# markokr/libacm

Measured on AMD Instinct MI355X. Metric: decoded PCM Msamples/sec over a batch of ACM streams (hot path on HBM-resident staged input), higher is better.
Workload: dtype int32

## Files before the change

libacm_amd/csrc/acm_kernels.hip:

```cpp
#include <hip/hip_runtime.h>

#include <utility>

#include "acm_device.h"
#include "acm_late_scale.h"
#include "acm_kernel_geo.h"

#ifndef ACM_L14_GROUPS
#define ACM_L14_GROUPS 3, 3, 3, 3, 2
#endif
#ifndef ACM_L13_GROUPS
#define ACM_L13_GROUPS 2, 3, 3, 3, 2
#endif

#ifndef ACM_OUT_F32
#define ACM_OUT_F32 0
#endif
#if ACM_OUT_F32
#define ACM_K_EMIT acm_sw_emit_f32
#define ACM_K_SMALL acm_small_level_f32
#define ACM_K_FUSED acm_fused_tile_f32
#define ACM_K_TILE2 acm_f32_tile2
#define ACM_K_CHUNK acm_f32_chunk
#define ACMK_OUT(name) name##_f32
// ... 1950 lines not shown
	struct Desc { uint32_t e[NE]; };
	struct Tables {
		v4i_t coef[3][NM][64];
		int32_t bias[3][2][QN];
		int32_t rsum[3][QN];
	};

	static __device__ __forceinline__ void fill_tables(Tables &t, const int tid, const int nthreads)
	{
		constexpr int32_t ONE = 1 << OutScale<L>::SHIFT;
		for (int k = tid; k < 3 * NM * 64; k += nthreads) {
			const int j = k / (NM * 64), mt = (k / 64) % NM, lane = k % 64;
			t.coef[j][mt][lane] = *reinterpret_cast<const v4i_t *>(&ACM_TZ6[VARIANT][j][16 * mt + (lane & 15)][16 * (lane >> 4)]);
		}
		for (int k = tid; k < 3 * 2 * QN; k += nthreads) {
			const int var = k / (2 * QN), par = (k / QN) & 1, q = k % QN;
			t.bias[var][par][q] = par ? 0 : ACM_TZ6_BIAS[VARIANT][var][q] * ONE;
		}
		for (int k = tid; k < 3 * QN; k += nthreads) {
			int32_t sum = 0;
			for (int c = 0; c < 64; c++)
				sum += ACM_TZ6[VARIANT][k / QN][k % QN][c];
			t.rsum[k / QN][k % QN] = 128 * sum;
		}
	}

	static __device__ __forceinline__ Desc fetch_desc(const uint32_t *__restrict__ pairs, const AcmTile2 &r)
	{
		Desc d;
		const uint32_t at = __builtin_amdgcn_readfirstlane((uint32_t)r.idx_off);
#pragma unroll
		for (int j = 0; j < NE; j++)
			d.e[j] = pairs[at + j];
		return d;
	}

	static __device__ __forceinline__ uint32_t entry_of(const Desc &d, const uint32_t u)
	{
		uint32_t e = (uint32_t)opaque_s((int32_t)d.e[0]);
#pragma unroll
		for (int j = 1; j < NE; j++)
			e = (u >> 1) >= (uint32_t)j ? (uint32_t)opaque_s((int32_t)d.e[j]) : e;
		return e;
	}

	template <int CTRL, int BANKS>
	static __device__ __forceinline__ v4u_t dpp4(const v4u_t old, const v4u_t src)
	{
		v4u_t r;
#pragma unroll
		for (int v = 0; v < 4; v++)
			r[v] = (uint32_t)__builtin_amdgcn_update_dpp((int)old[v], (int)src[v], CTRL, 0xF, BANKS, false);
		return r;
	}
	static constexpr int DPP_W0_BANKS = (1 << (SIGMA / 4)) - 1;
	static __device__ __forceinline__ void hand_history_on(Raw &raw)
	{
#pragma unroll
		for (int k = 0; k < 2; k++) {
			raw.lo[0][k] = dpp4<0x100 + (16 - SIGMA), DPP_W0_BANKS>(raw.lo[0][k], raw.lo[0][k + NSW]);
			raw.hi[0][k] = dpp4<0x100 + (16 - SIGMA), DPP_W0_BANKS>(raw.hi[0][k], raw.hi[0][k + NSW]);
		}
	}
	static __device__ __forceinline__ void take_history_from_partner(Raw &raw)
	{
#pragma unroll
		for (int k = 0; k < 2; k++) {
			raw.lo[0][k] = dpp4<0x110 + SIGMA, 0xF & ~DPP_W0_BANKS>(raw.lo[0][k], raw.lo[0][k + NSW]);
			raw.hi[0][k] = dpp4<0x110 + SIGMA, 0xF & ~DPP_W0_BANKS>(raw.hi[0][k], raw.hi[0][k + NSW]);
		}
	}
	static constexpr int JM = (TR & 1) ? 1 : TR / 2;
	static_assert(JM + 1 <= NE, "entries in reach are entries fetched");
	static __device__ __forceinline__ uint32_t half_bytes(const uint32_t cls) { return (0x4234u >> (4u * cls)) & 15u; }
	template <int J0>
	static __device__ __forceinline__ uint32_t mode_of(const uint32_t flags, const Desc &d, const uint32_t sval)
	{
		const uint32_t cls = d.e[0] & 3u;
		const uint32_t pair_units = (uint32_t)(COLS / 64) * half_bytes(cls);
		bool ok = (flags & ACM_TILE_ONEBLOCK) != 0 && cls != 0u;
		if constexpr (OutScale<L>::SHIFT != 0)
			ok = ok && sval < 65536u;
#pragma unroll
		for (int j = 1; j <= JM; j++)
			ok = ok && (d.e[j] & 3u) == cls;
#pragma unroll
		for (int j = J0; j < JM; j++)
			ok = ok && (d.e[j + 1] >> 2) - (d.e[j] >> 2) == pair_units;
		return ok ? (cls == ACMHIP_BP_NIB12 ? 3u : cls - (ACMHIP_BP_BYTE - 1u)) : 0u;
	}

#ifndef ACM_K3_LD_MOD
#define ACM_K3_LD_MOD " nt"
#endif
	template <bool KEEP>
	static __device__ __forceinline__ void issue(Raw &raw, const uint8_t *arena, const Desc &d, const int lane, const uint32_t odd, const uint32_t mode)
	{
		static_assert(!KEEP || KEEPS_ROWS, "the rows in front belong to another lane");
		constexpr int K0 = KEEP ? 2 : 0, J0 = KEEP ? 1 : 0;
		const uint32_t i = (uint32_t)lane & 15u, ks = (uint32_t)lane >> 4;
		const uint32_t c = class_of(i), rr = RR == 1 ? 0u : i / SIGMA;
		const uint32_t smode = __builtin_amdgcn_readfirstlane(mode);
		uint32_t va[NX][NG], vh[NX][NG];
		const uint8_t *sb[NX][NG];
		if (mode) {
			const uint32_t hb = smode == 1u ? 2u : smode == 2u ? 4u : 3u;
			const uint64_t base = reinterpret_cast<uint64_t>(arena) + ((uint64_t)(d.e[J0] >> 2) << 6);
			const uint32_t vl = (rr * (uint32_t)(NSW * COLS / 2) + c * (uint32_t)(QN / 2)) * hb + 16u * ks;
			const uint32_t vlh = vl - (smode == 3u ? 8u * ks : 0u);
#pragma unroll
			for (int k = K0; k < NX; k++)
#pragma unroll
				for (int g = 0; g < NG; g++) {
					va[k][g] = vl;
					vh[k][g] = vlh;
					sb[k][g] = sgpr_u64(base + (uint64_t)((((TR & 1 ? odd : 0u) + (uint32_t)(k - K0)) * (uint32_t)(COLS / 2) + group_at(g) * (uint32_t)(QN / 2)) * hb));
				}
		} else {
			const uint32_t e0 = d.e[0];
			const uint8_t *base = sgpr_u64(reinterpret_cast<uint64_t>(arena) + ((uint64_t)(e0 >> 2) << 6));
#pragma unroll
			for (int k = K0; k < NX; k++) {
				const uint32_t u = (TR & 1 ? odd : 0u) + rr * NSW + k;
				const uint32_t e = entry_of(d, u);
				const uint32_t hb = half_bytes(e & 3u);
				const uint32_t row_at = (((e >> 2) - (e0 >> 2)) << 6) + ((u & 1u) ? (uint32_t)(COLS / 2) * hb : 0u) + 16u * ks;
#pragma unroll
				for (int g = 0; g < NG; g++) {
					va[k][g] = row_at + (group_at(g) + c) * (uint32_t)(QN / 2) * hb;
					vh[k][g] = va[k][g] - ((e & 3u) == ACMHIP_BP_NIB12 ? 8u * ks : 0u);
					sb[k][g] = base;
				}
			}
		}
#pragma unroll
		for (int k = K0; k < NX; k++)
#pragma unroll
			for (int g = 0; g < NG; g++) {
				if constexpr (KEEPS_ROWS) {
					asm volatile("global_load_dwordx4 %0, %1, %2" ACM_K3_LD_MOD : "=v"(raw.lo[g][k]) : "v"(va[k][g]), "s"(sb[k][g]) : "memory");
					asm volatile("s_cmp_eq_u32 %3, 1\n\ts_cbranch_scc1 .Lacm_z8_%=\n\t"
						     "global_load_dwordx4 %0, %1, %2 offset:64" ACM_K3_LD_MOD "\n"
						     ".Lacm_z8_%=:"
						     : "+v"(raw.hi[g][k]) : "v"(vh[k][g]), "s"(sb[k][g]), "s"(smode) : "memory", "scc");
				} else {
					asm volatile("global_load_dwordx4 %0, %1, %2" : "=v"(raw.lo[g][k]) : "v"(va[k][g]), "s"(sb[k][g]) : "memory");
					asm volatile("s_cmp_eq_u32 %3, 1\n\ts_cbranch_scc1 .Lacm_z8_%=\n\t"
						     "global_load_dwordx4 %0, %1, %2 offset:64\n"
						     ".Lacm_z8_%=:"
						     : "+v"(raw.hi[g][k]) : "v"(vh[k][g]), "s"(sb[k][g]), "s"(smode) : "memory", "scc");
				}
			}
	}
	static __device__ __forceinline__ v4u_t expand_nib(const v4u_t x)
	{
		const uint32_t M = 0xF0F0F0F0u;
		return v4u_t{ x[0] & M, (x[0] << 4) & M, x[1] & M, (x[1] << 4) & M };
	}
	static __device__ __forceinline__ v4u_t sra4(const v4u_t x)
	{
		v4u_t r;
#pragma unroll
		for (int v = 0; v < 4; v++) {
			const uint32_t m = x[v] & 0x80808080u;
			r[v] = ((x[v] >> 4) & 0x0F0F0F0Fu) | ((m << 1) - (m >> 3));
		}
		return r;
	}
	static __device__ __forceinline__ v4u_t shl4(const v4u_t x)
	{
		return v4u_t{ (x[0] << 4) & 0xF0F0F0F0u, (x[1] << 4) & 0xF0F0F0F0u, (x[2] << 4) & 0xF0F0F0F0u, (x[3] << 4) & 0xF0F0F0F0u };
	}
	static __device__ __forceinline__ void shift_history(Raw &raw)
	{
#pragma unroll
		for (int g = 0; g < NG; g++)
#pragma unroll
			for (int k = 0; k < 2; k++) {
				raw.lo[g][k] = raw.lo[g][k + NSW];
				raw.hi[g][k] = raw.hi[g][k + NSW];
			}
	}
	static __device__ __forceinline__ void zero_history(Raw &raw)
	{
		const v4u_t z = { 0, 0, 0, 0 };
#pragma unroll
		for (int g = 0; g < NG; g++)
#pragma unroll
			for (int k = 0; k < 2; k++)
				raw.lo[g][k] = raw.hi[g][k] = z;
	}

	static __device__ __forceinline__ v4i_t mfma(const v4u_t data, const v4i_t coef, const v4i_t acc)
	{
		return __builtin_amdgcn_mfma_i32_16x16x64_i8((v4i_t)data, coef, acc, 0, 0, 0);
	}

	static __device__ __forceinline__ int32_t opaque_s(int32_t v)
	{
		asm("" : "+s"(v));
		return v;
	}
	static __device__ __forceinline__ int32_t opaque_v(int32_t v)
	{
		asm("" : "+v"(v));
		return v;
	}

	template <bool WORDS, bool FAST, bool NIB = false>
	static __device__ __forceinline__ void run_t(const Raw &raw, uint32_t *const tile, const Tables &t, const int lane, const uint32_t hvs,
						     const uint32_t in_front, const uint32_t sval, const bool wordu = false, const Desc *dd = nullptr,
						     const uint32_t odd = 0u, const bool nform = false)
	{
		static_assert(!NIB || (WORDS && FAST), "rows in N form are a fast-path matter; the general path takes them to bytes first");
		const v4i_t zero = { 0, 0, 0, 0 };
		const uint32_t h = (uint32_t)lane >> 4, qd = (uint32_t)lane & 15u;
		uint32_t c0[NH], rrd[NH];
		uint32_t o_lane[NH];
#pragma unroll
		for (int hf = 0; hf < NH; hf++) {
			const uint32_t i = 4u * h + (uint32_t)(hf * NVH);
			c0[hf] = RR == 1 ? class_of(i) : i % SIGMA;
			rrd[hf] = RR == 1 ? 0u : i / SIGMA;
			const uint32_t m_lane = rrd[hf] * (uint32_t)(NSW * COLS) + c0[hf] + (uint32_t)SIGMA * qd;
			o_lane[hf] = m_lane + (m_lane >> PS);
		}
		uint32_t bias_at[NSW][NH];
		int32_t val[NSW][NH], dv2[NSW][NH], dv1[NSW][NH];
		bool step2[NSW], step1[NSW];
		bool small[NSW];
#pragma unroll
		for (int s = 0; s < NSW; s++)
			small[s] = OutScale<L>::SHIFT == 0;
		if constexpr (FAST) {
#pragma unroll
			for (int s = 0; s < NSW; s++) {
				step2[s] = step1[s] = false;
				small[s] = true;
#pragma unroll
				for (int hf = 0; hf < NH; hf++)
					val[s][hf] = dv2[s][hf] = dv1[s][hf] = 0;
			}
		} else if constexpr (RR <= 2) {
			int32_t rowval[TR + 2];
#pragma unroll
			for (int k = 0; k < TR + 2; k++)
				rowval[k] = (int32_t)__builtin_amdgcn_readlane(hvs, k);
#pragma unroll
			for (int s = 0; s < NSW; s++) {
				const int32_t a0 = rowval[s + 2], a1 = rowval[s + 1], a2 = rowval[s];
				if constexpr (RR == 1) {
					val[s][0] = a0;
					dv2[s][0] = a1 - a0;
					dv1[s][0] = a2 - a1;
					step2[s] = a1 != a0;
					step1[s] = a2 != a1;
					small[s] = (uint32_t)a0 < 65536u;
				} else {
					const int32_t b0 = rowval[NSW + s + 2], b1 = rowval[NSW + s + 1], b2 = rowval[NSW + s];
					val[s][0] = rrd[0] ? b0 : a0;
					dv2[s][0] = rrd[0] ? b1 - b0 : a1 - a0;
					dv1[s][0] = rrd[0] ? b2 - b1 : a2 - a1;
					step2[s] = a1 != a0 || b1 != b0;
					step1[s] = a2 != a1 || b2 != b1;
					small[s] = (uint32_t)(a0 | b0) < 65536u;
				}
			}
		} else {
			const uint32_t first = (uint32_t)__builtin_amdgcn_readfirstlane(hvs);
			const bool one_val = __builtin_amdgcn_ballot_w64(lane < TR + 2 && hvs != first) == 0;
#pragma unroll
			for (int s = 0; s < NSW; s++)
				step2[s] = step1[s] = false;
#pragma unroll
			for (int hf = 0; hf < NH; hf++) {
				int32_t g[NSW + 2];
#pragma unroll
				for (int k = 0; k < NSW + 2; k++)
					g[k] = one_val ? (int32_t)first : __builtin_amdgcn_ds_bpermute((int)(4u * (rrd[hf] * NSW + (uint32_t)k)), (int32_t)hvs);
#pragma unroll
				for (int s = 0; s < NSW; s++) {
					val[s][hf] = g[s + 2];
					dv2[s][hf] = g[s + 1] - g[s + 2];
					dv1[s][hf] = g[s] - g[s + 1];
					if (!one_val) {
						step2[s] = step2[s] || __builtin_amdgcn_ballot_w64(dv2[s][hf] != 0) != 0;
						step1[s] = step1[s] || __builtin_amdgcn_ballot_w64(dv1[s][hf] != 0) != 0;
					}
				}
			}
		}
#pragma unroll
		for (int s = 0; s < NSW; s++)
#pragma unroll
			for (int hf = 0; hf < NH; hf++) {
				const uint32_t row = in_front + rrd[hf] * NSW + s;
				bias_at[s][hf] = ((row < 2 ? row : 2u) * 2u + (c0[hf] == 0 ? 0u : 1u)) * (uint32_t)QN + qd;
			}
		const v4i_t *cf = &t.coef[0][0][lane];
		const auto &hi = raw.hi;
#ifndef ACM_K3_MT_UNROLL
#define ACM_K3_MT_UNROLL 1
#endif
#define ACM_PRAGMA_(x) _Pragma(#x)
#define ACM_UNROLL(n) ACM_PRAGMA_(unroll n)
		ACM_UNROLL(ACM_K3_MT_UNROLL)
		for (int mt = 0; mt < NM; mt++) {
			const v4i_t cf0 = cf[0], cf1 = cf[NM * 64], cf2 = cf[2 * NM * 64];
#pragma unroll
			for (int e = 0; e < NSET; e++) {
				const int g = e / NSW, s = e % NSW;
				int32_t b[NH];
#pragma unroll
				for (int hf = 0; hf < NH; hf++)
					b[hf] = g == 0 ? (&t.bias[0][0][0])[bias_at[s][hf] + 16u * (uint32_t)mt] : 0;
				const v4i_t l1 = mfma(raw.lo[g][s], cf2, zero);
				const v4i_t l2 = mfma(raw.lo[g][s + 1], cf1, l1);
				const v4i_t la = mfma(raw.lo[g][s + 2], cf0, l2);
				v4i_t y;
				if constexpr (FAST) {
					const int32_t sv = opaque_s((int32_t)__builtin_amdgcn_readfirstlane(sval));
#pragma unroll
					for (int v = 0; v < 4; v++)
						y[v] = __mul24(la[v], sv) + (v % NVH == 0 ? b[v / NVH] : 0);
					if constexpr (WORDS) {
						const v4i_t h1 = mfma(hi[g][s], cf2, zero);
						const v4i_t h2 = mfma(hi[g][s + 1], cf1, h1);
						const v4i_t ha = mfma(hi[g][s + 2], cf0, h2);
						if constexpr (NIB) {
							const int32_t sv4 = opaque_s((int32_t)__builtin_amdgcn_readfirstlane(sval << 4));
#pragma unroll
							for (int v = 0; v < 4; v++)
								y[v] = __mul24(ha[v], sv4) + y[v];
						} else {
							const uint32_t sv8 = (uint32_t)opaque_s((int32_t)__builtin_amdgcn_readfirstlane(sval << 8));
#pragma unroll
							for (int v = 0; v < 4; v++)
								y[v] = (int32_t)(__umul24((uint32_t)ha[v], sv8) + (uint32_t)y[v]);
						}
					}
				} else {
#pragma unroll
				for (int v = 0; v < 4; v++)
					y[v] = __mul24(la[v], val[s][v / NVH]) + (v % NVH == 0 ? b[v / NVH] : 0);
				if (step2[s]) {
#pragma unroll
					for (int v = 0; v < 4; v++)
						y[v] += __mul24(l2[v], dv2[s][v / NVH]);
				}
				if (step1[s]) {
#pragma unroll
					for (int v = 0; v < 4; v++)
						y[v] += __mul24(l1[v], dv1[s][v / NVH]);
				}
				if constexpr (WORDS && NH == 1) {
					if (wordu) {
						const int32_t *rs = &t.rsum[0][0] + 16 * mt + (int)qd;
						bool urow[3];
#pragma unroll
						for (int j = 0; j < 3; j++)
							urow[j] = (entry_of(*dd, (TR & 1 ? odd : 0u) + rrd[0] * NSW + (uint32_t)(s + j)) & 3u) == ACMHIP_BP_WORDU;
						const int32_t v0 = val[s][0], v1 = v0 + dv2[s][0], v2 = v1 + dv1[s][0];
						const int32_t add = __mul24(urow[2] ? v0 : 0, rs[0]) + __mul24(urow[1] ? v1 : 0, rs[QN]) + __mul24(urow[0] ? v2 : 0, rs[2 * QN]);
#pragma unroll
						for (int v = 0; v < 4; v++)
							y[v] += add;
					}
				}
				if constexpr (WORDS) {
					const v4i_t h1 = mfma(hi[g][s], cf2, zero);
					const v4i_t h2 = mfma(hi[g][s + 1], cf1, h1);
					const v4i_t ha = mfma(hi[g][s + 2], cf0, h2);
					{
						if (small[s] && !step2[s] && !step1[s] && !nform) {
							uint32_t v8[NH];
#pragma unroll
							for (int hf = 0; hf < NH; hf++)
								v8[hf] = (uint32_t)opaque_v((int32_t)((uint32_t)val[s][hf] << 8));
#pragma unroll
							for (int v = 0; v < 4; v++)
								y[v] = (int32_t)(__umul24((uint32_t)ha[v], v8[v / NVH]) + (uint32_t)y[v]);
							goto joined;
						}
					}
					{
					v4i_t yh;
					int32_t wv[NH], w2[NH], w1[NH];
#pragma unroll
					for (int hf = 0; hf < NH; hf++) {
						wv[hf] = opaque_v(val[s][hf]);
						w2[hf] = opaque_v(dv2[s][hf]);
						w1[hf] = opaque_v(dv1[s][hf]);
					}
#pragma unroll
					for (int v = 0; v < 4; v++)
						yh[v] = __mul24(ha[v], wv[v / NVH]);
					if (step2[s]) {
#pragma unroll
						for (int v = 0; v < 4; v++)
							yh[v] += __mul24(h2[v], w2[v / NVH]);
					}
					if (step1[s]) {
#pragma unroll
						for (int v = 0; v < 4; v++)
							yh[v] += __mul24(h1[v], w1[v / NVH]);
					}
					const uint32_t hs = nform ? 4u : 8u;
#pragma unroll
					for (int v = 0; v < 4; v++)
						y[v] = (int32_t)(((uint32_t)opaque_v(yh[v]) << hs) + (uint32_t)y[v]);
					}
				joined:;
				}
				}
				static_assert(COLS % (1 << PS) == 0 && (SIGMA * 16) % (1 << PS) == 0 &&
					      (NG == 1 || (group_at(NG - 1) % (1 << PS) + CB + 7 < (1 << PS) && SIGMA % (1 << PS) == 0)), "address split");
#pragma unroll
				for (int hf = 0; hf < NH; hf++) {
					uint32_t *const o = tile + (o_lane[hf] + (uint32_t)((s * COLS + ((s * COLS) >> PS)) + (group_at(g) + (group_at(g) >> PS))));
#pragma unroll
					for (int v = 0; v < NVH; v++)
						o[v] = (uint32_t)y[hf * NVH + v];
				}
			}
			cf += 64;
#pragma unroll
			for (int hf = 0; hf < NH; hf++)
				o_lane[hf] += SIGMA * 16 + ((SIGMA * 16) >> PS);
		}
	}

	static __device__ __forceinline__ void run(Raw &raw, uint32_t *const tile, const Tables &t, const int lane_, const uint32_t hvs,
						   const Desc &d, const uint32_t in_front, const uint32_t odd, const uint32_t mode, const uint32_t sval,
						   const bool first)
	{
#ifdef ACM_K3_OPAQUE_LANE
		const int lane = opaque_v(lane_);
#else
		const int lane = lane_;
#endif
		const bool all_new = !KEEPS_ROWS || first;
		if (mode == 3u) {
#pragma unroll
			for (int k = 0; k < NX; k++)
				if (k >= 2 || all_new) {
#pragma unroll
					for (int g = 0; g < NG; g++)
						raw.hi[g][k] = expand_nib(raw.hi[g][k]);
				}
			if constexpr (HISTORY_BY_DPP)
				take_history_from_partner(raw);
			run_t<true, true, true>(raw, tile, t, lane, 0u, in_front, sval);
			return;
		}
		if (mode) {
			if constexpr (HISTORY_BY_DPP)
				take_history_from_partner(raw);
			if (mode == 2u)
				run_t<true, true>(raw, tile, t, lane, 0u, in_front, sval);
			else
				run_t<false, true>(raw, tile, t, lane, 0u, in_front, sval);
			return;
		}
		uint32_t any_word = 0, any_nib = 0, any_wordu = 0;
#pragma unroll
		for (int j = 0; j < NE; j++) {
			any_word |= (d.e[j] & 3u) == ACMHIP_BP_WORD ? 1u : 0u;
			any_nib |= (d.e[j] & 3u) == ACMHIP_BP_NIB12 ? 1u : 0u;
			any_wordu |= (d.e[j] & 3u) == ACMHIP_BP_WORDU ? 1u : 0u;
		}
		any_word |= any_wordu;
		const uint32_t rr = RR == 1 ? 0u : ((uint32_t)lane & 15u) / SIGMA;
		if (any_nib) {
#pragma unroll
			for (int k = 0; k < NX; k++)
				if (k >= 2 || all_new) {
					if ((entry_of(d, (TR & 1 ? odd : 0u) + rr * NSW + k) & 3u) == ACMHIP_BP_NIB12) {
#pragma unroll
						for (int g = 0; g < NG; g++)
							raw.hi[g][k] = expand_nib(raw.hi[g][k]);
					}
				}
		}
		if constexpr (HISTORY_BY_DPP)
			take_history_from_partner(raw);
		const bool nform = any_nib && !any_word;
		if (any_word | any_nib) {
#pragma unroll
			for (int k = 0; k < NX; k++) {
				const uint32_t cls = entry_of(d, (TR & 1 ? odd : 0u) + rr * NSW + k) & 3u;
				const uint32_t mask = cls == ACMHIP_BP_BYTE ? 0u : 0xFFFFFFFFu;
#pragma unroll
				for (int g = 0; g < NG; g++)
					raw.hi[g][k] &= mask;
				if (any_nib && !nform && cls == ACMHIP_BP_NIB12) {
#pragma unroll
					for (int g = 0; g < NG; g++)
						raw.hi[g][k] = sra4(raw.hi[g][k]);
				}
			}
			run_t<true, false>(raw, tile, t, lane, hvs, in_front, 0u, any_wordu != 0, &d, odd, nform);
			if (any_nib && !nform && KEEPS_ROWS) {
#pragma unroll
				for (int k = NSW; k < NX; k++)
					if ((entry_of(d, (TR & 1 ? odd : 0u) + rr * NSW + k) & 3u) == ACMHIP_BP_NIB12) {
#pragma unroll
						for (int g = 0; g < NG; g++)
							raw.hi[g][k] = shl4(raw.hi[g][k]);
					}
			}
		} else {
			run_t<false, false>(raw, tile, t, lane, hvs, in_front, 0u);
		}
	}
};

template <int L_, int ABL, int... Gs>
__global__ void __launch_bounds__(64 * FirstPassZ<L_>::NW, 1)
ACM_K_CHUNK(const AcmTile2 *__restrict__ tiles, const uint32_t ntiles, const int16_t *__restrict__ idx, const uint32_t *__restrict__ pairs,
	  const acmhip_blkhdr *__restrict__ hdr, int16_t *__restrict__ pcm, int16_t *__restrict__ sink, const unsigned fmt,
	  uint32_t *__restrict__ claim, const uint32_t static_per, const uint32_t run_chunks, const uint32_t nclaimed)
{
	constexpr bool F32 = ACM_OUT_F32;

	using FP = FirstPassZ<L_>;
	using C = typename FP::C;
	constexpr int L = L_, COLS = C::COLS, NELEM = C::NELEM, TR = C::TR, NJ_LAST = C::NJ_LAST, NW = FP::NW;
	constexpr int WTILE = 8 + NELEM + (NELEM >> C::PS);
	constexpr int NCARRY_WORDS = carry_total<C, FP::G, Gs...>();
	constexpr int PASS_ABL = ABL | MODE_WAVE | (FP::NG > 1 && NW == 16 ? MODE_LEAN : 0);

	__shared__ uint32_t tile_mem[NW][WTILE];
	__shared__ uint32_t carry_all[NW][NCARRY_WORDS];
	__shared__ typename FP::Tables tables;

	const int lane0 = threadIdx.x & 63;
	const uint32_t wave = __builtin_amdgcn_readfirstlane(threadIdx.x >> 6);
	FP::fill_tables(tables, threadIdx.x, NW * 64);

	enum { SPLIT_CLAIM_LO, SPLIT_CLAIM_HI, SPLIT_WRAP, SPLIT_NCLAIMED, SPLIT_NSTATIC, SPLIT_RUN_CHUNKS, SPLIT_NTILES, SPLIT_WORDS };
	__shared__ __attribute__((aligned(8))) uint32_t split_mem[SPLIT_WORDS + 1];
	const uint32_t nvw = gridDim.x * NW, vw = blockIdx.x * NW + wave;
	const uint32_t per = nclaimed ? static_per : (ntiles + nvw - 1) / nvw;
	const uint32_t nstatic = nclaimed ? nvw * static_per : ntiles;
	if (threadIdx.x == 0) {
		const uint64_t c = nclaimed ? reinterpret_cast<uint64_t>(claim) : 0ull;
		split_mem[SPLIT_CLAIM_LO] = (uint32_t)c;
		split_mem[SPLIT_CLAIM_HI] = (uint32_t)(c >> 32);
		split_mem[SPLIT_WRAP] = nclaimed + nvw - 1;
		split_mem[SPLIT_NCLAIMED] = nclaimed;
		split_mem[SPLIT_NSTATIC] = nstatic;
		split_mem[SPLIT_RUN_CHUNKS] = run_chunks;
		split_mem[SPLIT_NTILES] = ntiles;
	}
	__syncthreads();

	uint32_t *const tile = tile_mem[wave] + 8;
	uint32_t *const carry_mem = carry_all[wave];

	uint32_t t = vw * per;
	uint32_t t_end = t + per < nstatic ? t + per : nstatic;
	if (t >= t_end) {
		if (!nclaimed)
			return;
		uint32_t k = 0;
		if (lane0 == 0)
			k = atomicInc(claim, nclaimed + nvw - 1);
		k = __builtin_amdgcn_readfirstlane(k);
		if (k >= nclaimed)
			return;
		t = nstatic + k * run_chunks;
		t_end = t + run_chunks < ntiles ? t + run_chunks : ntiles;
	}
	auto claim_next = [&](uint32_t v, const uint32_t more) -> uint32_t {
		uint64_t exec_was, at;
		asm volatile("s_cmp_lg_u32 %[more], 0\n\ts_cbranch_scc1 .Lacm_cl_%=\n\t"
			     "s_mov_b64 %[was], exec\n\ts_mov_b64 exec, 1\n\t"
			     "v_mov_b32 %[v], %[lds]\n\t"
			     "ds_read_b64 %[at], %[v]\n\tds_read_b32 %[v], %[v] offset:8\n\t"
			     "s_waitcnt lgkmcnt(0)\n\t"
			     "v_cmp_ne_u64 vcc, 0, %[at]\n\ts_cbranch_vccz .Lacm_cn_%=\n\t"
			     "global_atomic_inc %[v], %[at], %[v], off sc0\n"
			     ".Lacm_cn_%=:\n\t"
			     "s_mov_b64 exec, %[was]\n"
			     ".Lacm_cl_%=:"
			     : [v] "+v"(v), [was] "=&s"(exec_was), [at] "=&v"(at)
			     : [lds] "s"((uint32_t)reinterpret_cast<uintptr_t>((const __attribute__((address_space(3))) uint32_t *)&split_mem[SPLIT_CLAIM_LO])), [more] "s"(__builtin_amdgcn_readfirstlane(more))
			     : "memory", "scc", "vcc");
		return v;
	};
	static_assert(SPLIT_CLAIM_HI == SPLIT_CLAIM_LO + 1 && SPLIT_WRAP == SPLIT_CLAIM_LO + 2, "the claim statement reads these three as it finds them");
	auto split_word = [&](const int k) -> uint32_t { return __builtin_amdgcn_readfirstlane(split_mem[k]); };

	auto rows_in_front = [](const AcmTile2 &r) -> uint32_t { return (r.flags & ACM_TILE_FRESH) ? 0u : (r.flags & ACM_TILE_ROW1) ? 1u : 2u; };
	auto fetch_val = [&](const AcmTile2 &r, const int lane, uint32_t v, const uint32_t mode) -> uint32_t {
		const uint32_t *p = &hdr[0].val;
		if (!mode) {
			const uint32_t lr_fetch = (uint32_t)(lane < TR + 2 ? lane : TR + 1);
			const uint32_t missing = 2u - rows_in_front(r);
			const uint32_t q = r.rowpos + (lr_fetch < missing ? 0u : lr_fetch - missing);
			const uint32_t b = r.magic ? __umulhi(q, r.magic) : q;
			p = &hdr[r.hdr_blk + b].val;
		}
		asm volatile("s_cmp_lg_u32 %2, 0\n\ts_cbranch_scc1 .Lacm_zv_%=\n\t"
			     "global_load_dword %0, %1, off\n"
			     ".Lacm_zv_%=:"
			     : "+v"(v) : "v"(p), "s"(__builtin_amdgcn_readfirstlane(mode)) : "memory", "scc");
		return v;
	};
	typedef const uint32_t __attribute__((address_space(4))) *const_u32_ptr;
	auto val_of = [&](const AcmTile2 &r) -> uint32_t {
		const uint64_t a = reinterpret_cast<uint64_t>(&hdr[__builtin_amdgcn_readfirstlane(r.hdr_blk)].val);
		return *(const_u32_ptr)a << OutScale<L>::SHIFT;
	};

	constexpr int NVEC = TR * COLS / 8, PER_OWNER = NJ_LAST / 8, NSTORE = NVEC / 64;
	static_assert(NVEC % 64 == 0, "whole rounds");
	const uint8_t *const arena = reinterpret_cast<const uint8_t *>(idx);
	auto record_at = [&](const uint32_t k) -> AcmTile2 { return tiles[__builtin_amdgcn_readfirstlane(k < t_end ? k : t_end - 1)]; };
	constexpr int MODE_J0 = FP::KEEPS_ROWS ? 1 : 0;
#ifdef ACM_K3_NO_FAST
	auto mode_of = [&](const AcmTile2 &, const typename FP::Desc &, const uint32_t) -> uint32_t { return 0u; };
#else
	auto mode_of = [&](const AcmTile2 &r, const typename FP::Desc &d, const uint32_t sval) -> uint32_t {
		return FP::template mode_of<MODE_J0>(r.flags, d, sval);
	};
#endif
#ifdef ACM_STAMPS
	unsigned long long acc_[8] = { 0, 0, 0, 0, 0, 0, 0, 0 };
	unsigned long long wave_c0_, wave_r0_;
	stamp_both(wave_c0_, wave_r0_);
	unsigned long long last_ = wave_c0_;
	uint32_t wave_chunks_ = 0, wave_runs_ = 0;
#endif
	uint32_t claimed = 0;
	for (;;) {
		bool discard = false;
		{
			const uint32_t f0 = tiles[__builtin_amdgcn_readfirstlane(t)].flags;
			if (f0 & ACM_TILE_DISCARD) {
				discard = true;
			} else if (!(f0 & ACM_TILE_FRESH)) {
				discard = true;
				t--;
			}
		}
		AcmTile2 cur = record_at(t);
		typename FP::Desc dcur = FP::fetch_desc(pairs, cur);
		typename FP::Raw raw;
		{
			const v4u_t z = { 0, 0, 0, 0 };
#pragma unroll
			for (int g = 0; g < FP::NG; g++)
#pragma unroll
				for (int k = 0; k < FP::NX; k++)
					raw.hi[g][k] = z;
		}
		uint32_t mode_cur = 0u, sv_cur = val_of(cur);
		int lane_run = lane0;
		asm volatile("" : "+v"(lane_run));
		uint32_t hv = fetch_val(cur, lane_run, 0u, 0u);
		FP::template issue<false>(raw, arena, dcur, lane_run, (cur.flags & ACM_TILE_ODD) ? 1u : 0u, 0u);
		k2_wait<0>();
		bool fresh = true, first_of_run = true;
		AcmTile2 nxt = record_at(t + 1), nx2 = record_at(t + 2);
		typename FP::Desc dnxt = FP::fetch_desc(pairs, nxt);
		uint32_t sv_nxt = val_of(nxt);
		uint32_t mode_nxt = mode_of(nxt, dnxt, sv_nxt);
		ACM_STAMP(4);
#ifdef ACM_STAMPS
		wave_runs_++;
#endif
		for (;;) {
			const uint32_t tn = t + 1;
			const bool more = tn < t_end;
#ifdef ACM_STAMPS
			wave_chunks_++;
#endif
			int lane = lane0;
#ifdef ACM_K3_OPAQUE_LANE
			asm volatile("" : "+v"(lane));
#endif
			if (fresh)
				for (int k = lane; k < NCARRY_WORDS; k += 64)
					carry_mem[k] = 0u;
			const uint32_t hvs = hv << OutScale<L>::SHIFT;
			ACM_STAMP(0);
			phase_prio<true, PRIO_FIRST_PASS>();
			FP::run(raw, tile, tables, lane, hvs, dcur, rows_in_front(cur), (cur.flags & ACM_TILE_ODD) ? 1u : 0u, mode_cur, sv_cur, first_of_run);
			first_of_run = false;
			phase_prio<true, PRIO_IDLE>();
			ACM_STAMP(1);

			hv = fetch_val(nxt, lane, hv, mode_nxt);
			if constexpr (FP::HISTORY_IN_REGISTERS) {
				FP::shift_history(raw);
				if (nxt.flags & ACM_TILE_FRESH)
					FP::zero_history(raw);
				FP::template issue<true>(raw, arena, dnxt, lane, (nxt.flags & ACM_TILE_ODD) ? 1u : 0u, mode_nxt);
			} else if constexpr (FP::HISTORY_BY_DPP) {
				FP::hand_history_on(raw);
				if (nxt.flags & ACM_TILE_FRESH)
					FP::zero_history(raw);
				FP::template issue<true>(raw, arena, dnxt, lane, (nxt.flags & ACM_TILE_ODD) ? 1u : 0u, mode_nxt);
			} else {
				FP::template issue<false>(raw, arena, dnxt, lane, (nxt.flags & ACM_TILE_ODD) ? 1u : 0u, mode_nxt);
			}
			claimed = claim_next(claimed, more ? 1u : 0u);
			const AcmTile2 nx3 = record_at(t + 3);
			const typename FP::Desc dnx2 = FP::fetch_desc(pairs, nx2);
			const uint32_t sv_nx2 = val_of(nx2);
			ACM_STAMP(2);
			phase_prio<true, PRIO_LDS_PASSES>();
			run_lds_passes<C, PASS_ABL, true, FP::G, Gs...>(tile, lane, F32 ? (unsigned)ACMHIP_FMT_S16LE : fmt, carry_mem);
			tile_barrier<MODE_WAVE>();
			ACM_STAMP(3);
			if constexpr (F32) {
				float *out = discard ? reinterpret_cast<float *>(sink) : reinterpret_cast<float *>(pcm) + cur.pcm_off;
				lean_store_f32<C, 64, NSTORE, ABL>(tile, lane, out);
			} else {
				typedef uint32_t v4u __attribute__((ext_vector_type(4)));
				v4u *out = discard ? reinterpret_cast<v4u *>(sink) : reinterpret_cast<v4u *>(reinterpret_cast<uint16_t *>(pcm) + cur.pcm_off);
#pragma unroll
				for (int k = 0; k < NSTORE; k++) {
					const int vec = lane + k * 64;
					const uint32_t *q = tile + lds_at<C::PS>((vec / PER_OWNER) * NJ_LAST) + (vec % PER_OWNER) * park_piece<NJ_LAST>();
					const v4u o = { q[0], q[1], q[2], q[3] };
#ifdef ACM_K3_ST_MOD
					asm volatile("global_store_dwordx4 %0, %1, %2" ACM_K3_ST_MOD :: "v"((uint32_t)(vec * 16)), "v"(o), "s"(sgpr_u64(reinterpret_cast<uint64_t>(out))) : "memory");
#else
					__builtin_nontemporal_store(o, &out[vec]);
#endif
				}
			}
			ACM_STAMP(5);
			phase_prio<true, PRIO_IDLE>();
			k2_wait<F32 ? 2 * NSTORE : NSTORE>();
			ACM_STAMP(6);
			tile_barrier<MODE_WAVE>();
			if (!more)
				break;
			fresh = (nxt.flags & (ACM_TILE_FRESH | ACM_TILE_DISCARD)) != 0;
			discard = (nxt.flags & ACM_TILE_DISCARD) != 0;
			cur = nxt;
			dcur = dnxt;
			sv_cur = sv_nxt;
			mode_cur = mode_nxt;
			t = tn;
			nxt = nx2;
			dnxt = dnx2;
			sv_nxt = sv_nx2;
			mode_nxt = mode_of(nxt, dnxt, sv_nxt);
			nx2 = nx3;
		}
		const uint32_t k = __builtin_amdgcn_readfirstlane(claimed);
		if (k >= split_word(SPLIT_NCLAIMED))
			break;
		const uint32_t run = split_word(SPLIT_RUN_CHUNKS), end = split_word(SPLIT_NTILES);
		t = split_word(SPLIT_NSTATIC) + k * run;
		t_end = t + run < end ? t + run : end;
	}
#ifdef ACM_STAMPS
	if (lane0 == 0 && vw < 2048)
		for (int k = 0; k < 8; k++)
			g_acm_stamps[vw][k] = acc_[k];
	if (lane0 == 0 && vw < ACM_WAVE_STAMPS_MAX) {
		unsigned long long c1, r1;
		stamp_both(c1, r1);
		unsigned long long *const o = g_acm_wave_stamps[vw];
		o[0] = wave_c0_, o[1] = wave_r0_, o[2] = c1, o[3] = r1, o[4] = wave_chunks_, o[5] = stamp_where(), o[6] = wave_runs_, o[7] = 0;
	}
#endif
}

using acm_geo::Tile2Build;
using acm_geo::Tile2MBuild;
typedef void (*Tile2Fn)(const AcmTile2 *, uint32_t, const int16_t *, const uint32_t *, const acmhip_blkhdr *, int16_t *, int16_t *, unsigned);
template <class B, int... Gs>
constexpr Tile2Fn entry_k2()
{
	return ACM_K_TILE2<typename B::C, B::W, 0, false, Gs...>;
}
#ifdef ACM_ABLATION
template <int ABL>
constexpr Tile2Fn abl_k2() { return ACM_K_TILE2<Tile2Build<9>::C, Tile2Build<9>::W, ABL, false, 3, 3, 3>; }
const struct { int mask; Tile2Fn fn; } g_tile2_abl[] = {
	{ 1, abl_k2<1>() }, { 2, abl_k2<2>() }, { 4, abl_k2<4>() }, { 6, abl_k2<6>() }, { 8, abl_k2<8>() }, { 16, abl_k2<16>() },
	{ 17, abl_k2<17>() }, { 23, abl_k2<23>() }, { 32, abl_k2<32>() }, { 25, abl_k2<25>() }, { 31, abl_k2<31>() }, { 12, abl_k2<12>() },
};
#endif
const Tile2Fn g_tile2[ACM_K2_MAX_LEVEL - ACM_K2_MIN_LEVEL + 1] = {
	entry_k2<Tile2Build<6>, 2, 2, 2>(),
	entry_k2<Tile2Build<7>, 3, 2, 2>(),
	entry_k2<Tile2Build<8>, 3, 3, 2>(),
	entry_k2<Tile2Build<9>, 3, 3, 3>(),
	entry_k2<Tile2Build<10>, 3, 3, 2, 2>(),
	entry_k2<Tile2Build<11>, 3, 3, 3, 2>(),
	entry_k2<Tile2Build<12>, 3, 3, 3, 3>(),
	entry_k2<Tile2Build<13>, ACM_L13_GROUPS>(),
	entry_k2<Tile2Build<14>, ACM_L14_GROUPS>(),
};
template <class B, int... Gs>
constexpr Tile2Fn entry_k2m()
{
	return ACM_K_TILE2<typename B::C, B::W, 0, true, B::G0, Gs...>;
}
#ifndef ACM_K2M_L11_GROUPS
#define ACM_K2M_L11_GROUPS 3, 2, 2
#endif
#ifndef ACM_K2M_L12_GROUPS
#define ACM_K2M_L12_GROUPS 3, 3, 2
#endif
#ifndef ACM_K2M_L13_GROUPS
#define ACM_K2M_L13_GROUPS 3, 3, 3
#endif
#ifndef ACM_K3_L13_GROUPS
// ... 560 lines not shown
```

Before: 1.470 million.

## Fully unroll L9 fast mt loop with flat LDS store offsets and hoisted DPP history

For the L==9 fast path, the mt loop is fully unrolled, with a sched_barrier placed at the top of each iteration. LDS store addresses now come from a few precomputed opaque base registers plus constant offsets kept under 256, so each store can use an immediate offset instead of its own address arithmetic. The run dispatcher is also reorganised so that take_history_from_partner is called once on a single path before branching on mode, and the general path moves into run_general. The aim is fewer VALU address computations and less code duplication, at the cost of longer code and possibly higher register pressure.

```diff
diff --git a/libacm_amd/csrc/acm_kernels.hip b/libacm_amd/csrc/acm_kernels.hip
--- a/libacm_amd/csrc/acm_kernels.hip
+++ b/libacm_amd/csrc/acm_kernels.hip
@@ -2276,10 +2276,26 @@
 #ifndef ACM_K3_MT_UNROLL
 #define ACM_K3_MT_UNROLL 1
 #endif
-#define ACM_PRAGMA_(x) _Pragma(#x)
-#define ACM_UNROLL(n) ACM_PRAGMA_(unroll n)
-		ACM_UNROLL(ACM_K3_MT_UNROLL)
+#ifndef ACM_K3_MT_FLAT
+#define ACM_K3_MT_FLAT 1
+#endif
+		constexpr bool MT_FLAT = FAST && ACM_K3_MT_FLAT && L == 9;
+		constexpr int MT_UNROLL = MT_FLAT ? NM : ACM_K3_MT_UNROLL;
+		constexpr uint32_t O_STEP = SIGMA * 16 + ((SIGMA * 16) >> PS), O_REACH = 256 - NVH;
+		constexpr uint32_t O_SPAN = (NM - 1) * O_STEP + (NSW - 1) * (COLS + (COLS >> PS)) + group_at(NG - 1) + (group_at(NG - 1) >> PS);
+		constexpr int NBASE = MT_FLAT ? (int)(O_SPAN / O_REACH) + 1 : 1;
+		uint32_t o_base[NH][NBASE];
+		if constexpr (MT_FLAT) {
+#pragma unroll
+			for (int hf = 0; hf < NH; hf++)
+#pragma unroll
+				for (int k = 0; k < NBASE; k++)
+					o_base[hf][k] = (uint32_t)opaque_v((int32_t)(o_lane[hf] + (uint32_t)k * O_REACH));
+		}
+#pragma unroll MT_UNROLL
 		for (int mt = 0; mt < NM; mt++) {
+			if constexpr (MT_FLAT)
+				__builtin_amdgcn_sched_barrier(0);
 			const v4i_t cf0 = cf[0], cf1 = cf[NM * 64], cf2 = cf[2 * NM * 64];
 #pragma unroll
 			for (int e = 0; e < NSET; e++) {
@@ -2391,7 +2407,9 @@
 					      (NG == 1 || (group_at(NG - 1) % (1 << PS) + CB + 7 < (1 << PS) && SIGMA % (1 << PS) == 0)), "address split");
 #pragma unroll
 				for (int hf = 0; hf < NH; hf++) {
-					uint32_t *const o = tile + (o_lane[hf] + (uint32_t)((s * COLS + ((s * COLS) >> PS)) + (group_at(g) + (group_at(g) >> PS))));
+					const uint32_t at = (uint32_t)((s * COLS + ((s * COLS) >> PS)) + (group_at(g) + (group_at(g) >> PS)));
+					const uint32_t flat_at = (uint32_t)mt * O_STEP + at;
+					uint32_t *const o = MT_FLAT ? tile + o_base[hf][flat_at / O_REACH] + flat_at % O_REACH : tile + (o_lane[hf] + at);
 #pragma unroll
 					for (int v = 0; v < NVH; v++)
 						o[v] = (uint32_t)y[hf * NVH + v];
@@ -2400,10 +2418,43 @@
 			cf += 64;
 #pragma unroll
 			for (int hf = 0; hf < NH; hf++)
-				o_lane[hf] += SIGMA * 16 + ((SIGMA * 16) >> PS);
-		}
-	}
-
+				o_lane[hf] += O_STEP;
+		}
+	}
+
+	static __device__ __forceinline__ void run_general(Raw &raw, uint32_t *const tile, const Tables &t, const int lane, const uint32_t hvs,
+							   const Desc &d, const uint32_t in_front, const uint32_t odd,
+							   const uint32_t any_word, const uint32_t any_nib, const uint32_t any_wordu, const uint32_t rr)
+	{
+		const bool nform = any_nib && !any_word;
+		if (any_word | any_nib) {
+#pragma unroll
+			for (int k = 0; k < NX; k++) {
+				const uint32_t cls = entry_of(d, (TR & 1 ? odd : 0u) + rr * NSW + k) & 3u;
+				const uint32_t mask = cls == ACMHIP_BP_BYTE ? 0u : 0xFFFFFFFFu;
+#pragma unroll
+				for (int g = 0; g < NG; g++)
+					raw.hi[g][k] &= mask;
+				if (any_nib && !nform && cls == ACMHIP_BP_NIB12) {
+#pragma unroll
+					for (int g = 0; g < NG; g++)
+						raw.hi[g][k] = sra4(raw.hi[g][k]);
+				}
+			}
+			run_t<true, false>(raw, tile, t, lane, hvs, in_front, 0u, any_wordu != 0, &d, odd, nform);
+			if (any_nib && !nform && KEEPS_ROWS) {
+#pragma unroll
+				for (int k = NSW; k < NX; k++)
+					if ((entry_of(d, (TR & 1 ? odd : 0u) + rr * NSW + k) & 3u) == ACMHIP_BP_NIB12) {
+#pragma unroll
+						for (int g = 0; g < NG; g++)
+							raw.hi[g][k] = shl4(raw.hi[g][k]);
+					}
+			}
+		} else {
+			run_t<false, false>(raw, tile, t, lane, hvs, in_front, 0u);
+		}
+	}
 	static __device__ __forceinline__ void run(Raw &raw, uint32_t *const tile, const Tables &t, const int lane_, const uint32_t hvs,
 						   const Desc &d, const uint32_t in_front, const uint32_t odd, const uint32_t mode, const uint32_t sval,
 						   const bool first)
@@ -2413,6 +2464,53 @@
 #else
 		const int lane = lane_;
 #endif
+		if constexpr (HISTORY_BY_DPP) {
+			const bool all_new = !KEEPS_ROWS || first;
+			uint32_t any_word = 0, any_nib = 0, any_wordu = 0;
+			const uint32_t rr = RR == 1 ? 0u : ((uint32_t)lane & 15u) / SIGMA;
+			if (mode == 3u) {
+#pragma unroll
+				for (int k = 0; k < NX; k++)
+					if (k >= 2 || all_new) {
+#pragma unroll
+						for (int g = 0; g < NG; g++)
+							raw.hi[g][k] = expand_nib(raw.hi[g][k]);
+					}
+			} else if (!mode) {
+#pragma unroll
+				for (int j = 0; j < NE; j++) {
+					any_word |= (d.e[j] & 3u) == ACMHIP_BP_WORD ? 1u : 0u;
+					any_nib |= (d.e[j] & 3u) == ACMHIP_BP_NIB12 ? 1u : 0u;
+					any_wordu |= (d.e[j] & 3u) == ACMHIP_BP_WORDU ? 1u : 0u;
+				}
+				any_word |= any_wordu;
+				if (any_nib) {
+#pragma unroll
+					for (int k = 0; k < NX; k++)
+						if (k >= 2 || all_new) {
+							if ((entry_of(d, (TR & 1 ? odd : 0u) + rr * NSW + k) & 3u) == ACMHIP_BP_NIB12) {
+#pragma unroll
+								for (int g = 0; g < NG; g++)
+									raw.hi[g][k] = expand_nib(raw.hi[g][k]);
+							}
+						}
+				}
+			}
+			take_history_from_partner(raw);
+			if (mode == 3u) {
+				run_t<true, true, true>(raw, tile, t, lane, 0u, in_front, sval);
+				return;
+			}
+			if (mode) {
+				if (mode == 2u)
+					run_t<true, true>(raw, tile, t, lane, 0u, in_front, sval);
+				else
+					run_t<false, true>(raw, tile, t, lane, 0u, in_front, sval);
+				return;
+			}
+			run_general(raw, tile, t, lane, hvs, d, in_front, odd, any_word, any_nib, any_wordu, rr);
+			return;
+		}
 		const bool all_new = !KEEPS_ROWS || first;
 		if (mode == 3u) {
 #pragma unroll
@@ -2422,14 +2520,10 @@
 					for (int g = 0; g < NG; g++)
 						raw.hi[g][k] = expand_nib(raw.hi[g][k]);
 				}
-			if constexpr (HISTORY_BY_DPP)
-				take_history_from_partner(raw);
 			run_t<true, true, true>(raw, tile, t, lane, 0u, in_front, sval);
 			return;
 		}
 		if (mode) {
-			if constexpr (HISTORY_BY_DPP)
-				take_history_from_partner(raw);
 			if (mode == 2u)
 				run_t<true, true>(raw, tile, t, lane, 0u, in_front, sval);
 			else
@@ -2456,36 +2550,7 @@
 					}
 				}
 		}
-		if constexpr (HISTORY_BY_DPP)
-			take_history_from_partner(raw);
-		const bool nform = any_nib && !any_word;
-		if (any_word | any_nib) {
-#pragma unroll
-			for (int k = 0; k < NX; k++) {
-				const uint32_t cls = entry_of(d, (TR & 1 ? odd : 0u) + rr * NSW + k) & 3u;
-				const uint32_t mask = cls == ACMHIP_BP_BYTE ? 0u : 0xFFFFFFFFu;
-#pragma unroll
-				for (int g = 0; g < NG; g++)
-					raw.hi[g][k] &= mask;
-				if (any_nib && !nform && cls == ACMHIP_BP_NIB12) {
-#pragma unroll
-					for (int g = 0; g < NG; g++)
-						raw.hi[g][k] = sra4(raw.hi[g][k]);
-				}
-			}
-			run_t<true, false>(raw, tile, t, lane, hvs, in_front, 0u, any_wordu != 0, &d, odd, nform);
-			if (any_nib && !nform && KEEPS_ROWS) {
-#pragma unroll
-				for (int k = NSW; k < NX; k++)
-					if ((entry_of(d, (TR & 1 ? odd : 0u) + rr * NSW + k) & 3u) == ACMHIP_BP_NIB12) {
-#pragma unroll
-						for (int g = 0; g < NG; g++)
-							raw.hi[g][k] = shl4(raw.hi[g][k]);
-					}
-			}
-		} else {
-			run_t<false, false>(raw, tile, t, lane, hvs, in_front, 0u);
-		}
+		run_general(raw, tile, t, lane, hvs, d, in_front, odd, any_word, any_nib, any_wordu, rr);
 	}
 };
 
```

New measurement: 1.462 million. About the same (-0.5%).
